# PaddlePaddle/MetaGym

Hardware: NVIDIA H100
Metric: env-steps/sec (quadrotor 6-DoF, 65k envs) (higher is better)
Workload: dtype f32

## Files before the change

### metagym_b200/csrc/quad.cu

```cuda
#include <math.h>
#include <stdlib.h>
#include <string.h>
#include <new>
#include <vector>

#include "mgb_common.cuh"
#include "quad_lanes.cuh"

namespace {

constexpr int kThreads = 64;
constexpr int kMaxObs = 19;

struct QuadConst {
    float h;
    float k1phi;
    float k1;
    float inv_phi;
    float hjm;
    float hk;
    float mm;
    float ct0, ct1, ct2;
    float vmin, vmax;
    float A[4], B[4];
    float px[4], py[4], pz[4];
    float Df[3], Dm[3];
    float cg[3];
    float hI[9];
    float gm;
    float c_hm;
    float c_h2m;
    float fail_r2, fail_v2, fail_w2;
    float dt, healthy, z_off;
    float init_v[3], init_w[3], noise_v, noise_w;
    int nt, task, substeps, obs_dim;
    int rk4_steps;
    float rk4_h;
    float inv_jm, inv_m;
    float Iinv[9];
    int simple;
};

struct QuadArgs {
    float4 *planes;
    int64_t n_pad;
    int64_t n;
    int64_t env_base;
    const float *act;
    float *obs;
    float *rew;
    uint8_t *done;
    int32_t *fail;
    float *final_obs;
    const float *targets;
    const int32_t *sat;
    int map_rows, map_cols, x_off, y_off;
    const int32_t *env2task;
    uint64_t seed;
    int auto_reset;
    int per_cta;
    int T;
    uint64_t act_seed;
    uint32_t t_base;
    float *act_out;
    MgbMirrors mir;
};

template <class T> struct VState {
    T p[3], v[3], om[3], w[4], R[9];
    int ct[Lanes<T>::N], ep[Lanes<T>::N];
};
using QState = VState<float>;

constexpr int kTileEnvs = 128;
constexpr int kPlanes = 6;

__device__ __forceinline__ float4 *tile_base(const QuadArgs &a, int64_t e)
{
    return a.planes + (e / kTileEnvs) * (kPlanes * kTileEnvs) + (e % kTileEnvs);
}

__device__ __forceinline__ void unpack_state(const float4 q[kPlanes], QState &s)
{
    s.p[0] = q[0].x; s.p[1] = q[0].y; s.p[2] = q[0].z; s.v[0] = q[0].w;
    s.v[1] = q[1].x; s.v[2] = q[1].y; s.om[0] = q[1].z; s.om[1] = q[1].w;
    s.om[2] = q[2].x; s.w[0] = q[2].y; s.w[1] = q[2].z; s.w[2] = q[2].w;
    s.w[3] = q[3].x; s.R[0] = q[3].y; s.R[1] = q[3].z; s.R[2] = q[3].w;
    s.R[3] = q[4].x; s.R[4] = q[4].y; s.R[5] = q[4].z; s.R[6] = q[4].w;
    s.R[7] = q[5].x; s.R[8] = q[5].y; s.ct[0] = __float_as_int(q[5].z); s.ep[0] = __float_as_int(q[5].w);
}
__device__ __forceinline__ void pack_state(const QState &s, float4 q[kPlanes])
{
    q[0] = make_float4(s.p[0], s.p[1], s.p[2], s.v[0]);
    q[1] = make_float4(s.v[1], s.v[2], s.om[0], s.om[1]);
    q[2] = make_float4(s.om[2], s.w[0], s.w[1], s.w[2]);
    q[3] = make_float4(s.w[3], s.R[0], s.R[1], s.R[2]);
    q[4] = make_float4(s.R[3], s.R[4], s.R[5], s.R[6]);
    q[5] = make_float4(s.R[7], s.R[8], __int_as_float(s.ct[0]), __int_as_float(s.ep[0]));
}

__device__ __forceinline__ void load_state(const QuadArgs &a, int64_t e, QState &s)
{
    const float4 *b = tile_base(a, e);
    float4 q[kPlanes];
#pragma unroll
    for (int k = 0; k < kPlanes; ++k) q[k] = b[k * kTileEnvs];
    unpack_state(q, s);
}

__device__ __forceinline__ void store_state(const QuadArgs &a, int64_t e, const QState &s)
{
    float4 *b = tile_base(a, e);
    float4 q[kPlanes];
    pack_state(s, q);
#pragma unroll
    for (int k = 0; k < kPlanes; ++k) b[k * kTileEnvs] = q[k];
}

template <class T> __device__ __forceinline__ void get_lane_state(const VState<T> &s, int h, QState &o);
template <class T> __device__ __forceinline__ void set_lane_state(VState<T> &s, int h, const QState &o);

__device__ __forceinline__ void load_state2(const QuadArgs &a, int64_t e, VState<f2> &s)
{
    QState s0, s1;
    load_state(a, e, s0);
    load_state(a, e + 1, s1);
    set_lane_state(s, 0, s0);
    set_lane_state(s, 1, s1);
}
__device__ __forceinline__ void store_state2(const QuadArgs &a, int64_t e, const VState<f2> &s)
{
    QState s0, s1;
    get_lane_state(s, 0, s0);
    get_lane_state(s, 1, s1);
    store_state(a, e, s0);
    store_state(a, e + 1, s1);
}
// ... 321 lines not shown
        for (int r = 0; r < 3; ++r) { acc.p[r] = fmaf(2.f, k.p[r], acc.p[r]); acc.v[r] = fmaf(2.f, k.v[r], acc.v[r]); acc.om[r] = fmaf(2.f, k.om[r], acc.om[r]); }
#pragma unroll
        for (int r = 0; r < 4; ++r) acc.w[r] = fmaf(2.f, k.w[r], acc.w[r]);
#pragma unroll
        for (int r = 0; r < 9; ++r) acc.R[r] = fmaf(2.f, k.R[r], acc.R[r]);
        quad_axpy(s, k, h, t);
        quad_rhs<SIMPLE>(c, t, kV, k);
#pragma unroll
        for (int r = 0; r < 3; ++r) { acc.p[r] += k.p[r]; acc.v[r] += k.v[r]; acc.om[r] += k.om[r]; }
#pragma unroll
        for (int r = 0; r < 4; ++r) acc.w[r] += k.w[r];
#pragma unroll
        for (int r = 0; r < 9; ++r) acc.R[r] += k.R[r];
        const int ct = s.ct[0], ep = s.ep[0];
        quad_axpy(s, acc, h * (1.0f / 6.0f), t);
        s = t; s.ct[0] = ct; s.ep[0] = ep;
        const float psq = sq3(s.p);
        const float vsq = sq3(s.v);
        const float osq = sq3(s.om);
        fail = fail_code(c, psq, vsq, osq);
        if (fail) break;
    }
    adjugate(s.R, adj, id);
    float pw = 0.f;
#pragma unroll
    for (int i = 0; i < 4; ++i) pw += fabsf(fmaf(-c.k1phi, s.w[i], kV[i]) * c.inv_phi * V[i]);
    power = pw;
    return fail;
}

template <class T>
__device__ __forceinline__ void observe(const QuadConst &c, const VState<T> &s, const T adj[9], T id, T *o, T bv[3],
                                        T Ri[9])
{
#pragma unroll
    for (int k = 0; k < 9; ++k) Ri[k] = vmul(adj[k], id);
#pragma unroll
    for (int r = 0; r < 3; ++r) {
        bv[r] = dot3(Ri[3 * r], s.v[0], Ri[3 * r + 1], s.v[1], Ri[3 * r + 2], s.v[2]);
        o[r] = bv[r];
        o[3 + r] = dot3(Ri[3 * r], s.p[0], Ri[3 * r + 1], s.p[1], Ri[3 * r + 2], s.p[2]);
        o[6 + r] = vmul(Ri[3 * r + 2], -9.8f);
        o[9 + r] = s.om[r];
    }
    o[12] = fast_atan2(vneg(s.R[6]), vsqrt(vfma(s.R[8], s.R[8], vmul(s.R[7], s.R[7]))));
    o[13] = fast_atan2(s.R[7], s.R[8]);
    o[14] = fast_atan2(s.R[3], s.R[0]);
    o[15] = vadd(s.p[2], c.z_off);
}

template <class T> __device__ __forceinline__ void reset_env(const QuadConst &c, VState<T> &s, int h, const double u[12])
{
#pragma unroll
    for (int k = 0; k < 3; ++k) {
        set_lane(s.p[k], h, 0.f);
        const double sv = u[k] > 0.5 ? 1.0 : -1.0, sw = u[6 + k] > 0.5 ? 1.0 : -1.0;
        set_lane(s.v[k], h, (float)((double)c.init_v[k] + ((double)c.noise_v * u[3 + k]) * sv));
        set_lane(s.om[k], h, (float)((double)c.init_w[k] + ((double)c.noise_w * u[9 + k]) * sw));
    }
#pragma unroll
    for (int k = 0; k < 4; ++k) set_lane(s.w[k], h, 0.f);
#pragma unroll
    for (int k = 0; k < 9; ++k) set_lane(s.R[k], h, (k % 4 == 0) ? 1.f : 0.f);
}

__device__ __forceinline__ void philox_reset_draws(uint64_t seed, int64_t genv, int ep, double u[12])
{
    const uint2 key = make_uint2((uint32_t)seed, (uint32_t)(seed >> 32));
#pragma unroll
    for (int j = 0; j < 3; ++j) {
        const uint4 r = mgb_philox4x32_10(
            make_uint4((uint32_t)genv, (uint32_t)((uint64_t)genv >> 32), (uint32_t)ep, MGB_STREAM_RESET + j), key);
        u[4 * j + 0] = (double)mgb_u01(r.x);
        u[4 * j + 1] = (double)mgb_u01(r.y);
        u[4 * j + 2] = (double)mgb_u01(r.z);
        u[4 * j + 3] = (double)mgb_u01(r.w);
    }
}

template <class T> struct TargetRows {
    T cur[3];
    T nxt[3];
};
template <class T>
__device__ __forceinline__ void prefetch_targets(const QuadConst &c, const float *trow, int ct, int h, TargetRows<T> &tr)
{
    const int t = ct < c.nt - 1 ? ct : c.nt - 1;
    const float *g = trow + 3 * (ct - 1), *q = trow + 3 * t;
    set_lane(tr.cur[0], h, __ldg(g)); set_lane(tr.cur[1], h, __ldg(g + 1)); set_lane(tr.cur[2], h, __ldg(g + 2));
    set_lane(tr.nxt[0], h, __ldg(q)); set_lane(tr.nxt[1], h, __ldg(q + 1)); set_lane(tr.nxt[2], h, __ldg(q + 2));
}

__device__ __forceinline__ int slice_bound(double v, int len)
{
    long long x = v < -2.0e9 ? -2000000000LL : (v > 2.0e9 ? 2000000000LL : (long long)v);
    if (x < 0) { x += len; if (x < 0) x = 0; }
    if (x > len) x = len;
    return (int)x;
}

__device__ __forceinline__ bool map_collision(const QuadArgs &a, float x_old, float y_old, float z_old, float x_new,
                                              float y_new, float z_new)
{
    const double xo = (double)x_old + a.x_off, xn = (double)x_new + a.x_off;
    const double yo = (double)y_old + a.y_off, yn = (double)y_new + a.y_off;
    const double x_min = floor(fmin(xo, xn)), x_max = ceil(fmax(xo, xn));
    const double y_min = floor(fmin(yo, yn)), y_max = ceil(fmax(yo, yn));
    const int z_lo = (int)floorf(fminf(z_old, z_new)), z_hi = (int)ceilf(fmaxf(z_old, z_new));
    const int ys = slice_bound(y_min, a.map_rows), ye = slice_bound(y_max + 1.0, a.map_rows);
    const int xs = slice_bound(x_min, a.map_cols), xe = slice_bound(x_max + 1.0, a.map_cols);
    int any = 0;
    if (ys < ye && xs < xe) {
        const int W = a.map_cols + 1;
        any = (a.sat[ye * W + xe] - a.sat[ys * W + xe] - a.sat[ye * W + xs] + a.sat[ys * W + xs]) > 0 ? 1 : 0;
    }
    return z_lo < any || z_hi < any;
}

template <class T>
__device__ __forceinline__ void observe_reset(const QuadConst &c, const QuadArgs &a, int64_t e, const VState<T> &s, int h,
                                              T *o)
{
    set_lane(o[0], h, lane(s.v[0], h)); set_lane(o[1], h, lane(s.v[1], h)); set_lane(o[2], h, lane(s.v[2], h));
    set_lane(o[3], h, 0.f); set_lane(o[4], h, 0.f); set_lane(o[5], h, 0.f);
    set_lane(o[6], h, 0.f * -9.8f); set_lane(o[7], h, 0.f * -9.8f); set_lane(o[8], h, -9.8f);
    set_lane(o[9], h, lane(s.om[0], h)); set_lane(o[10], h, lane(s.om[1], h)); set_lane(o[11], h, lane(s.om[2], h));
    set_lane(o[12], h, -0.f); set_lane(o[13], h, 0.f); set_lane(o[14], h, 0.f);
    set_lane(o[15], h, 0.f + c.z_off);
    if (c.task == MGB_TASK_VELOCITY_CONTROL) {
        const float *trow = a.targets + ((int64_t)a.env2task[e] * c.nt) * 3;
        const int t = s.ct[h] < c.nt - 1 ? s.ct[h] : c.nt - 1;
        set_lane(o[16], h, __ldg(trow + 3 * t)); set_lane(o[17], h, __ldg(trow + 3 * t + 1));
        set_lane(o[18], h, __ldg(trow + 3 * t + 2));
    }
}

template <class T>
__device__ __forceinline__ void finish_step(const QuadConst &c, const QuadArgs &a, int64_t e, VState<T> &s,
                                            const T adj[9], T id, T z_old, T x_old, T y_old, T power,
                                            const int fail[Lanes<T>::N], const TargetRows<T> &tr, T *o, T &reward,
                                            int done_flag[Lanes<T>::N], bool write_final[Lanes<T>::N])
{
    constexpr int N = Lanes<T>::N;
    T bv[3], Ri[9];
    observe(c, s, adj, id, o, bv, Ri);
    if (c.task == MGB_TASK_VELOCITY_CONTROL) {
        o[16] = tr.nxt[0]; o[17] = tr.nxt[1]; o[18] = tr.nxt[2];
    }
    reward = vneg(vmin(vmul(c.dt, power), bc<T>(c.healthy)));
    int done[N];
#pragma unroll
    for (int h = 0; h < N; ++h) done[h] = 0;
    if (c.task == MGB_TASK_VELOCITY_CONTROL) {
        const T g0 = tr.cur[0], g1 = tr.cur[1], g2 = tr.cur[2];
        T diff = bc<T>(0.f);
#pragma unroll
        for (int r = 0; r < 3; ++r) diff = vadd(diff, vabs(vsub(dot3(Ri[3 * r], g0, Ri[3 * r + 1], g1, Ri[3 * r + 2], g2), bv[r])));
        reward = vadd(reward, vmul(-0.001f, diff));
    } else {
        const T z_new = vadd(s.p[2], c.z_off);
        T bonus, vn, on;
        if (c.task == MGB_TASK_HOVERING_CONTROL) {
            vn = vsqrt(sq3(s.v));
            on = vsqrt(sq3(s.om));
        }
#pragma unroll
        for (int h = 0; h < N; ++h) {
            bool coll;
            if (a.sat) coll = map_collision(a, lane(x_old, h), lane(y_old, h), lane(z_old, h), lane(s.p[0], h),
                                            lane(s.p[1], h), lane(z_new, h));
            else coll = fminf(lane(z_old, h), lane(z_new, h)) < 0.f;
            float tr = coll ? 0.f : c.healthy;
            if (c.task == MGB_TASK_HOVERING_CONTROL) {
                tr -= lane(vn, h) + lane(on, h);
                const float zm = fabsf(0.f - lane(s.p[2], h));
                tr += zm < 0.5f ? 10.f : fmaxf(-20.f, 0.5f - zm);
            }
            set_lane(bonus, h, tr);
            if (coll) { done[h] = 1; s.ct[h] = 0; }
        }
        reward = vadd(reward, bonus);
    }
#pragma unroll
    for (int h = 0; h < N; ++h) {
        if (s.ct[h] == c.nt) { done[h] = 1; s.ct[h] = 0; }
        if (fail[h]) { done[h] = 1; s.ct[h] = 0; }
        done_flag[h] = done[h];
        write_final[h] = false;
        if (done[h] && a.auto_reset) {
            write_final[h] = true;
            s.ep[h] += 1;
            double u[12];
            philox_reset_draws(a.seed, a.env_base + e + h, s.ep[h], u);
            reset_env(c, s, h, u);
        }
    }
}

__device__ __forceinline__ void publish_tile(float *gobs, const float *tile, int64_t e0, int rows, int D)
{
    const uint32_t bytes = (uint32_t)rows * (uint32_t)D * 4u;
    float *dst = gobs + e0 * D;
    if ((bytes & 15u) == 0 && ((reinterpret_cast<uintptr_t>(dst) & 15u) == 0)) {
        mgb_fence_proxy_async();
        __syncthreads();
        if (threadIdx.x == 0) {
            mgb_bulk_store(dst, tile, bytes);
            mgb_bulk_commit();
        }
    } else {
        __syncthreads();
        for (int i = threadIdx.x; i < rows * D; i += blockDim.x) dst[i] = tile[i];
    }
}

__device__ __forceinline__ void publish_tile_mirrored(const MgbMirrors &m, float *gobs, const float *tile, int64_t e0,
                                                      int rows, int D)
{
    const uint32_t bytes = (uint32_t)rows * (uint32_t)D * 4u;
    float *dst = gobs + e0 * D;
    if ((bytes & 15u) == 0 && ((reinterpret_cast<uintptr_t>(dst) & 15u) == 0)) {
        mgb_fence_proxy_async();
        __syncthreads();
        if (threadIdx.x == 0) {
            mgb_bulk_store(dst, tile, bytes);
            mgb_mirror_bulk_store(m, dst, tile, bytes);
            mgb_bulk_commit();
        }
    } else {
        __syncthreads();
        for (int i = threadIdx.x; i < rows * D; i += blockDim.x) {
            dst[i] = tile[i];
            mgb_mirror_store(m, dst + i, tile[i]);
        }
    }
}

template <bool SIMPLE, bool EARLY, class T>
__device__ __forceinline__ void step_body(const QuadConst &c, const QuadArgs &a, int64_t e, int nact, VState<T> &s,
                                          const T V[4], float *trow, float *frow, int &final_mask)
{
    constexpr int N = Lanes<T>::N;
    const int D = c.obs_dim;
    T adj[9], id, power;
    adjugate(s.R, adj, id);
    TargetRows<T> tr;
    int ct_now[N];
#pragma unroll
    for (int h = 0; h < N; ++h) {
        s.ct[h] += 1;
        ct_now[h] = s.ct[h];
    }
    const bool vel = c.task == MGB_TASK_VELOCITY_CONTROL;
    if (EARLY && vel) {
#pragma unroll
        for (int h = 0; h < N; ++h) {
            const int64_t eh = h < nact ? e + h : e;
            prefetch_targets(c, a.targets + ((int64_t)__ldg(a.env2task + eh) * c.nt) * 3, ct_now[h], h, tr);
        }
    }
    const T z_old = vadd(s.p[2], c.z_off);
    const T x_old = s.p[0], y_old = s.p[1];
    int fail[N];
    if (N == 1 && c.rk4_steps > 0) {
        QState s1;
        get_lane_state(s, 0, s1);
        float adj1[9], id1, pw1;
        fail[0] = integrate_rk4<SIMPLE>(c, s1, make_float4(lane(V[0], 0), lane(V[1], 0), lane(V[2], 0), lane(V[3], 0)),
                                        adj1, id1, pw1);
        set_lane_state(s, 0, s1);
#pragma unroll
        for (int k = 0; k < 9; ++k) set_lane(adj[k], 0, adj1[k]);
        set_lane(id, 0, id1);
        set_lane(power, 0, pw1);
    } else {
        const bool failed = integrate<SIMPLE, T>(c, s, V, adj, id, power, fail);
        if (N > 1 && failed) {
#pragma unroll 1
            for (int h = 0; h < N; ++h) {
                QState s1;
                load_state(a, e + h, s1);
                float adj1[9], id1, pw1;
                adjugate(s1.R, adj1, id1);
                const float V1[4] = {lane(V[0], h), lane(V[1], h), lane(V[2], h), lane(V[3], h)};
                int f1[1];
                integrate<SIMPLE, float>(c, s1, V1, adj1, id1, pw1, f1);
                s1.ct[0] = s.ct[h];
                s1.ep[0] = s.ep[h];
                set_lane_state(s, h, s1);
#pragma unroll
                for (int k = 0; k < 9; ++k) set_lane(adj[k], h, adj1[k]);
                set_lane(id, h, id1);
                set_lane(power, h, pw1);
                fail[h] = f1[0];
            }
        }
    }
    if (!EARLY && vel) {
#pragma unroll
        for (int h = 0; h < N; ++h) {
            const int64_t eh = h < nact ? e + h : e;
            prefetch_targets(c, a.targets + ((int64_t)__ldg(a.env2task + eh) * c.nt) * 3, ct_now[h], h, tr);
        }
    }
    const bool state_first = N == 1 && !EARLY && vel;
    if (state_first) {
        QState s1;
        get_lane_state(s, 0, s1);
        if (s1.ct[0] == c.nt || fail[0]) s1.ct[0] = 0;
        store_state(a, e, s1);
    }
    T o[kMaxObs], reward;
    int done[N];
    bool wf[N];
    finish_step(c, a, e, s, adj, id, z_old, x_old, y_old, power, fail, tr, o, reward, done, wf);
    bool stored = false;
    if constexpr (N == 2) {
        if (nact == 2) {
            store_state2(a, e, s);
            *reinterpret_cast<float2 *>(a.rew + e) = reward.v;
            *reinterpret_cast<uchar2 *>(a.done + e) = make_uchar2((uint8_t)done[0], (uint8_t)done[1]);
            if (a.fail) *reinterpret_cast<int2 *>(a.fail + e) = make_int2(fail[0], fail[1]);
            stored = true;
        }
    }
    if (!stored) {
#pragma unroll
        for (int h = 0; h < N; ++h) {
            if (h < nact) {
                QState s1;
                get_lane_state(s, h, s1);
                if (!state_first || wf[h]) store_state(a, e + h, s1);
                a.rew[e + h] = lane(reward, h);
                a.done[e + h] = (uint8_t)done[h];
                if (a.fail) a.fail[e + h] = fail[h];
            }
        }
    }
#pragma unroll
    for (int h = 0; h < N; ++h) {
        if (h < nact) {
            float *tr_h = trow + h * D;
            if (wf[h]) {
                if (a.final_obs) {
                    float *fr_h = frow + h * D;
#pragma unroll
                    for (int k = 0; k < 16; ++k) fr_h[k] = lane(o[k], h);
                    if (D == 19) { fr_h[16] = lane(o[16], h); fr_h[17] = lane(o[17], h); fr_h[18] = lane(o[18], h); }
                    final_mask |= 1 << h;
                }
                observe_reset(c, a, e + h, s, h, o);
            }
#pragma unroll
            for (int k = 0; k < 16; ++k) tr_h[k] = lane(o[k], h);
            if (D == 19) { tr_h[16] = lane(o[16], h); tr_h[17] = lane(o[17], h); tr_h[18] = lane(o[18], h); }
        }
    }
}

__device__ __forceinline__ void publish_final(const QuadArgs &a, const float *ftile, int64_t e, int local_row, int lanes,
                                              int final_mask, int D)
{
    if (!a.final_obs) return;
    if (__syncthreads_or(final_mask)) {
        for (int h = 0; h < lanes; ++h) {
            if (final_mask & (1 << h)) {
                float *dst = a.final_obs + (e + h) * D;
                const float *frow = ftile + (local_row + h) * D;
                for (int k = 0; k < D; ++k) dst[k] = frow[k];
            }
        }
    }
}

template <bool SIMPLE>
__global__ void __launch_bounds__(kThreads) quad_step_kernel(const __grid_constant__ QuadConst c,
                                                             const __grid_constant__ QuadArgs a)
{
    __shared__ __align__(128) float tile[kThreads * kMaxObs];
    __shared__ __align__(128) float ftile[kThreads * kMaxObs];
    const int64_t e0 = (int64_t)blockIdx.x * kThreads;
    const int64_t e = e0 + threadIdx.x;
    const int rows = (int)((a.n - e0) < kThreads ? (a.n - e0) : kThreads);
    const int D = c.obs_dim;
    const bool active = e < a.n;
    int final_mask = 0;

    asm volatile("griddepcontrol.launch_dependents;");
    asm volatile("griddepcontrol.wait;" ::: "memory");

    if (active) {
        QState s;
        load_state(a, e, s);
        const float4 act = __ldg(reinterpret_cast<const float4 *>(a.act) + e);
        const float V[4] = {act.x, act.y, act.z, act.w};
        step_body<SIMPLE, false, float>(c, a, e, 1, s, V, tile + threadIdx.x * D, ftile + threadIdx.x * D, final_mask);
    }
    publish_tile(a.obs, tile, e0, rows, D);
    publish_final(a, ftile, e, threadIdx.x, 1, final_mask, D);
    if (threadIdx.x == 0) mgb_bulk_wait_read<0>();
}

template <bool SIMPLE>
__global__ void __launch_bounds__(512, 1) quad_step_wide_kernel(const __grid_constant__ QuadConst c,
                                                                const __grid_constant__ QuadArgs a)
{
    extern __shared__ __align__(128) float wide_smem[];
    const int per = a.per_cta;
    float *tile = wide_smem, *ftile = wide_smem + (size_t)per * kMaxObs;
    const int64_t e0 = (int64_t)blockIdx.x * per;
    const int64_t e = e0 + threadIdx.x;
    int rows = (int)((a.n - e0) < per ? (a.n - e0) : per);
    if (rows < 0) rows = 0;
    const int D = c.obs_dim;
    const bool active = (int)threadIdx.x < rows;
    int final_mask = 0;
    asm volatile("griddepcontrol.launch_dependents;");
    asm volatile("griddepcontrol.wait;" ::: "memory");
    if (active) {
        QState s;
        load_state(a, e, s);
        const float4 act = __ldg(reinterpret_cast<const float4 *>(a.act) + e);
        const float V[4] = {act.x, act.y, act.z, act.w};
        step_body<SIMPLE, true, float>(c, a, e, 1, s, V, tile + threadIdx.x * D, ftile + threadIdx.x * D, final_mask);
    }
    if (rows > 0) publish_tile(a.obs, tile, e0, rows, D);
    else __syncthreads();
    publish_final(a, ftile, e, threadIdx.x, 1, final_mask, D);
    if (threadIdx.x == 0) mgb_bulk_wait_read<0>();
}

template <bool SIMPLE>
__global__ void __launch_bounds__(256, 1) quad_step2_kernel(const __grid_constant__ QuadConst c,
                                                            const __grid_constant__ QuadArgs a)
{
    extern __shared__ __align__(128) float pair_smem[];
    const int per = a.per_cta;
    float *tile = pair_smem, *ftile = pair_smem + (size_t)per * kMaxObs;
    const int64_t e0 = (int64_t)blockIdx.x * per;
    int rows = (int)((a.n - e0) < per ? (a.n - e0) : per);
    if (rows < 0) rows = 0;
    const int le = 2 * (int)threadIdx.x;
    const int64_t e = e0 + le;
    const int D = c.obs_dim;
    const int nact = rows - le >= 2 ? 2 : (rows - le > 0 ? 1 : 0);
    int final_mask = 0;
    asm volatile("griddepcontrol.launch_dependents;");
    asm volatile("griddepcontrol.wait;" ::: "memory");
    if (nact > 0) {
        VState<f2> s;
        load_state2(a, e, s);
        const float4 a0 = __ldg(reinterpret_cast<const float4 *>(a.act) + e);
        const float4 a1 = nact == 2 ? __ldg(reinterpret_cast<const float4 *>(a.act) + e + 1) : make_float4(0.f, 0.f, 0.f, 0.f);
        const f2 V[4] = {pack2(a0.x, a1.x), pack2(a0.y, a1.y), pack2(a0.z, a1.z), pack2(a0.w, a1.w)};
        step_body<SIMPLE, true, f2>(c, a, e, nact, s, V, tile + le * D, ftile + le * D, final_mask);
    }
    if (rows > 0) publish_tile(a.obs, tile, e0, rows, D);
    else __syncthreads();
    publish_final(a, ftile, e, le, 2, final_mask, D);
    if (threadIdx.x == 0) mgb_bulk_wait_read<0>();
}

constexpr int kStreamThreads = 128;

template <bool SIMPLE>
__global__ void __launch_bounds__(kStreamThreads, 4) quad_stream_kernel(const __grid_constant__ QuadConst c,
                                                                        const __grid_constant__ QuadArgs a)
{
    __shared__ __align__(128) float4 stage[2][7][kStreamThreads];
    __shared__ __align__(128) float tile[kStreamThreads * kMaxObs];
    __shared__ __align__(128) float ftile[kStreamThreads * kMaxObs];
    __shared__ __align__(8) uint64_t full[2];
    const int D = c.obs_dim;
    const int64_t n_tiles = (a.n + kStreamThreads - 1) / kStreamThreads;
    const int tid = threadIdx.x;

    asm volatile("griddepcontrol.launch_dependents;");
    asm volatile("griddepcontrol.wait;" ::: "memory");
    if (tid == 0) {
        mgb_mbar_init(&full[0], 1);
        mgb_mbar_init(&full[1], 1);
        mgb_fence_mbar_init();
    }
    __syncthreads();

    auto fetch = [&](int64_t t, int st) {
        const int64_t e0 = t * kStreamThreads;
        const uint32_t rows = (uint32_t)((a.n - e0) < kStreamThreads ? (a.n - e0) : kStreamThreads);
        static_assert(kStreamThreads == kTileEnvs, "one CTA iteration = one state tile");
        mgb_mbar_expect_tx(&full[st], 6u * kTileEnvs * 16u + rows * 16u);
        mgb_bulk_load(stage[st][0], a.planes + t * (6 * kTileEnvs), 6u * kTileEnvs * 16u, &full[st]);
        mgb_bulk_load(stage[st][6], reinterpret_cast<const float4 *>(a.act) + e0, rows * 16u, &full[st]);
    };

    int64_t t = blockIdx.x;
    if (tid == 0 && t < n_tiles) fetch(t, 0);
    uint32_t phase[2] = {0u, 0u};
    int st = 0;
    for (; t < n_tiles; t += gridDim.x, st ^= 1) {
        const int64_t t_next = t + gridDim.x;
        if (tid == 0 && t_next < n_tiles) fetch(t_next, st ^ 1);
        mgb_mbar_wait(&full[st], phase[st]);
        phase[st] ^= 1u;
        const int64_t e0 = t * kStreamThreads, e = e0 + tid;
        const int rows = (int)((a.n - e0) < kStreamThreads ? (a.n - e0) : kStreamThreads);
        int final_mask = 0;
        if (tid == 0) mgb_bulk_wait_read<0>();
        __syncthreads();
        if (tid < rows) {
            QState s;
            float4 q[kPlanes];
#pragma unroll
            for (int k = 0; k < kPlanes; ++k) q[k] = stage[st][k][tid];
            unpack_state(q, s);
            const float4 act = stage[st][6][tid];
            const float V[4] = {act.x, act.y, act.z, act.w};
            step_body<SIMPLE, true, float>(c, a, e, 1, s, V, tile + tid * D, ftile + tid * D, final_mask);
        }
        publish_tile(a.obs, tile, e0, rows, D);
        publish_final(a, ftile, e, tid, 1, final_mask, D);
        __syncthreads();
    }
    if (tid == 0) mgb_bulk_wait_read<0>();
}

template <bool SIMPLE, int XM>
__global__ void __launch_bounds__(kThreads, 8) quad_rollout_kernel(const __grid_constant__ QuadConst c,
                                                                const __grid_constant__ QuadArgs a)
{
    __shared__ __align__(128) float tiles[2][kThreads * kMaxObs];
    const int64_t e0 = (int64_t)blockIdx.x * kThreads;
    const int64_t e = e0 + threadIdx.x;
    const int rows = (int)((a.n - e0) < kThreads ? (a.n - e0) : kThreads);
    const int D = c.obs_dim;
    const bool active = e < a.n;
    QState s;
    float adj[9], id = 1.f;
    if (active) {
        load_state(a, e, s);
        adjugate(s.R, adj, id);
    }
    const uint2 akey = make_uint2((uint32_t)a.act_seed, (uint32_t)(a.act_seed >> 32));
    const int64_t genv = a.env_base + e;
    const float *trow = nullptr;
    if (active && c.task == MGB_TASK_VELOCITY_CONTROL) trow = a.targets + ((int64_t)__ldg(a.env2task + e) * c.nt) * 3;
    float4 act_next = make_float4(0.f, 0.f, 0.f, 0.f);
    if (active && a.act) act_next = __ldg(reinterpret_cast<const float4 *>(a.act) + e);
    for (int t = 0; t < a.T; ++t) {
        float *tile = tiles[t & 1];
        if (threadIdx.x == 0) mgb_bulk_wait_read<1>();
        __syncthreads();
        uint32_t done_byte = 0;
        if (active) {
            float4 act;
            if (a.act) {
                act = act_next;
                if (t + 1 < a.T) act_next = __ldg(reinterpret_cast<const float4 *>(a.act) + (int64_t)(t + 1) * a.n + e);
            } else {
                const uint4 r = mgb_philox4x32_10(make_uint4((uint32_t)genv, (uint32_t)((uint64_t)genv >> 32),
                                                             a.t_base + (uint32_t)t, MGB_STREAM_ACTION),
                                                  akey);
                const float span = c.vmax - c.vmin;
                act = make_float4(fmaf(span, mgb_u01(r.x), c.vmin), fmaf(span, mgb_u01(r.y), c.vmin),
                                  fmaf(span, mgb_u01(r.z), c.vmin), fmaf(span, mgb_u01(r.w), c.vmin));
                if (a.act_out) {
                    float4 *ap = reinterpret_cast<float4 *>(a.act_out) + (int64_t)t * a.n + e;
                    if (XM == 2) mgb_mc_st(mgb_shift(ap, a.mir.delta[0]), act);
                    else *ap = act;
                    if (XM == 1) mgb_mirror_store(a.mir, ap, act);
                }
            }
            s.ct[0] += 1;
            TargetRows<float> tr;
            if (c.task == MGB_TASK_VELOCITY_CONTROL) prefetch_targets(c, trow, s.ct[0], 0, tr);
            const float z_old = s.p[2] + c.z_off;
            const float x_old = s.p[0], y_old = s.p[1];
            float power;
            int fail[1];
            fail[0] = integrate1<SIMPLE>(c, s, act, adj, id, power);
            float o[kMaxObs], reward;
            int done[1];
            bool wf[1];
            finish_step<float>(c, a, e, s, adj, id, z_old, x_old, y_old, power, fail, tr, o, reward, done, wf);
            if (wf[0]) {
                observe_reset(c, a, e, s, 0, o);
                adjugate(s.R, adj, id);
            }
            if (a.rew) {
                if (XM == 2) mgb_mc_st(mgb_shift(a.rew + (int64_t)t * a.n + e, a.mir.delta[0]), reward);
                else a.rew[(int64_t)t * a.n + e] = reward;
                if (XM == 1) mgb_mirror_store(a.mir, a.rew + (int64_t)t * a.n + e, reward);
            }
            done_byte = (uint32_t)done[0];
            if (a.done && XM != 2) {
                a.done[(int64_t)t * a.n + e] = (uint8_t)done[0];
                if (XM == 1) mgb_mirror_store(a.mir, a.done + (int64_t)t * a.n + e, (uint8_t)done[0]);
            }
            if (a.obs) {
                float *orow = tile + threadIdx.x * D;
#pragma unroll
                for (int k = 0; k < 16; ++k) orow[k] = o[k];
                if (D == 19) { orow[16] = o[16]; orow[17] = o[17]; orow[18] = o[18]; }
            }
        }
        if (XM == 2) {
            if (a.done) mgb_mc_st_bytes(mgb_shift(a.done + (int64_t)t * a.n + e, a.mir.delta[0]), done_byte, active);
            if (a.obs) {
                __syncthreads();
                mgb_mc_copy_tile(mgb_shift(a.obs + ((int64_t)t * a.n + e0) * D, a.mir.delta[0]), tile,
                                 (uint32_t)rows * (uint32_t)D * 4u);
            }
        } else if (a.obs) {
            if (XM == 1) publish_tile_mirrored(a.mir, a.obs + (int64_t)t * a.n * D, tile, e0, rows, D);
            else publish_tile(a.obs + (int64_t)t * a.n * D, tile, e0, rows, D);
        }
    }
    if (active) store_state(a, e, s);
    if (threadIdx.x == 0) mgb_bulk_wait_read<0>();
}

__global__ void __launch_bounds__(kThreads) quad_reset_kernel(const __grid_constant__ QuadConst c,
                                                              const __grid_constant__ QuadArgs a,
                                                              const uint8_t *__restrict__ mask,
                                                              const double *__restrict__ noise)
{
    const int64_t e = (int64_t)blockIdx.x * kThreads + threadIdx.x;
    if (e >= a.n) return;
    QState s;
    load_state(a, e, s);
    if (!mask || mask[e]) {
        double u[12];
        if (noise) {
#pragma unroll
            for (int k = 0; k < 12; ++k) u[k] = noise[e * 12 + k];
        } else {
            s.ep[0] += 1;
            philox_reset_draws(a.seed, a.env_base + e, s.ep[0], u);
        }
        reset_env(c, s, 0, u);
        store_state(a, e, s);
    }
    if (a.obs) {
        float adj[9], id, o[kMaxObs], bv[3], Ri[9];
        adjugate(s.R, adj, id);
        observe(c, s, adj, id, o, bv, Ri);
        if (c.task == MGB_TASK_VELOCITY_CONTROL) {
            const float *trow = a.targets + ((int64_t)a.env2task[e] * c.nt) * 3;
            const int t = s.ct[0] < c.nt - 1 ? s.ct[0] : c.nt - 1;
            o[16] = trow[3 * t]; o[17] = trow[3 * t + 1]; o[18] = trow[3 * t + 2];
        }
        float *dst = a.obs + e * c.obs_dim;
#pragma unroll
        for (int k = 0; k < 16; ++k) dst[k] = o[k];
        if (c.obs_dim == 19) { dst[16] = o[16]; dst[17] = o[17]; dst[18] = o[18]; }
    }
}

__global__ void quad_state_kernel(QuadArgs a, float *state, int32_t *ct, int load)
{
    const int64_t e = (int64_t)blockIdx.x * blockDim.x + threadIdx.x;
    if (e >= a.n) return;
    QState s;
    load_state(a, e, s);
    float *row = state + e * 22;
    if (load) {
        for (int k = 0; k < 3; ++k) { s.p[k] = row[k]; s.v[k] = row[3 + k]; s.om[k] = row[6 + k]; }
        for (int k = 0; k < 4; ++k) s.w[k] = row[9 + k];
        for (int k = 0; k < 9; ++k) s.R[k] = row[13 + k];
        if (ct) s.ct[0] = ct[e];
        store_state(a, e, s);
    } else {
        for (int k = 0; k < 3; ++k) { row[k] = s.p[k]; row[3 + k] = s.v[k]; row[6 + k] = s.om[k]; }
        for (int k = 0; k < 4; ++k) row[9 + k] = s.w[k];
        for (int k = 0; k < 9; ++k) row[13 + k] = s.R[k];
        if (ct) ct[e] = s.ct[0];
    }
}

__global__ void quad_init_kernel(QuadArgs a)
{
    const int64_t e = (int64_t)blockIdx.x * blockDim.x + threadIdx.x;
    if (e >= a.n_pad) return;
    QState s;
    for (int k = 0; k < 3; ++k) s.p[k] = s.v[k] = s.om[k] = 0.f;
    for (int k = 0; k < 4; ++k) s.w[k] = 0.f;
    for (int k = 0; k < 9; ++k) s.R[k] = (k % 4 == 0) ? 1.f : 0.f;
    s.ct[0] = 0;
    s.ep[0] = 0;
    store_state(a, e, s);
}

template <bool SIMPLE>
__global__ void quad_targets_kernel(const __grid_constant__ QuadConst c, const float *__restrict__ act, int n_tasks,
                                    float *__restrict__ tbl)
{
    const int k = blockIdx.x * blockDim.x + threadIdx.x;
    if (k >= n_tasks) return;
    QState s;
    for (int q = 0; q < 3; ++q) s.p[q] = s.v[q] = s.om[q] = 0.f;
    for (int q = 0; q < 4; ++q) s.w[q] = 0.f;
    for (int q = 0; q < 9; ++q) s.R[q] = (q % 4 == 0) ? 1.f : 0.f;
    s.ct[0] = 0; s.ep[0] = 0;
    float adj[9], id, power;
    adjugate(s.R, adj, id);
    for (int t = 0; t < c.nt; ++t) {
        const float4 a4 = reinterpret_cast<const float4 *>(act)[(int64_t)k * c.nt + t];
        const int fail = integrate1<SIMPLE>(c, s, a4, adj, id, power);
        float *dst = tbl + ((int64_t)k * c.nt + t) * 3;
        dst[0] = s.v[0]; dst[1] = s.v[1]; dst[2] = s.v[2];
        if (fail) {
            for (int r = t + 1; r < c.nt; ++r) {
                float *d2 = tbl + ((int64_t)k * c.nt + r) * 3;
                d2[0] = d2[1] = d2[2] = __int_as_float(0x7fc00000);
            }
            return;
        }
    }
}

}

struct mgb_quad {
    int device = 0;
    int64_t n = 0, n_pad = 0, env_base = 0;
    mgb_quad_cfg cfg;
    QuadConst c;
    float4 *planes = nullptr;
    int32_t *sat = nullptr;
    int map_rows = 0, map_cols = 0, x_off = 0, y_off = 0;
    float *targets = nullptr;
    int32_t *env2task = nullptr;
    int n_tasks = 0;
    int auto_reset = 0;
    int num_sms = 132;
    int wide_kernel = -1;
    int packed = 0;
    int stream_kernel = 1;
    int pdl = 1;
    int zerocopy = 1;
    uint64_t seed = 0;
    uint32_t t_base = 0;
    int64_t launches = 0;
    MgbMirrors mir = {};
    MgbMirrorWindow mir_win;
    float *h_act = nullptr, *h_obs = nullptr, *h_rew = nullptr, *h_final = nullptr;
    uint8_t *h_done = nullptr;
    int32_t *h_fail = nullptr;
    float *d_act = nullptr, *d_obs = nullptr, *d_rew = nullptr, *d_final = nullptr;
    uint8_t *d_done = nullptr;
    int32_t *d_fail = nullptr;
};

static QuadArgs base_args(const mgb_quad *h)
{
    QuadArgs a;
    memset(&a, 0, sizeof(a));
    a.planes = h->planes;
    a.n_pad = h->n_pad;
    a.n = h->n;
    a.env_base = h->env_base;
    a.targets = h->targets;
    a.sat = h->sat; a.map_rows = h->map_rows; a.map_cols = h->map_cols; a.x_off = h->x_off; a.y_off = h->y_off;
    a.env2task = h->env2task;
    a.seed = h->seed;
    a.auto_reset = h->auto_reset;
    return a;
}

static int derive_constants(const mgb_quad_cfg *g, QuadConst *c)
{
    memset(c, 0, sizeof(*c));
    c->h = (float)g->precision;
    c->k1 = (float)(g->phi / g->ra);
    c->k1phi = (float)(g->phi / g->ra * g->phi);
    c->inv_phi = (float)(1.0 / g->phi);
    c->hjm = (float)(g->precision / g->jm);
    c->hk = (float)(g->precision / g->jm * (g->phi / g->ra * g->phi));
    c->mm = (float)g->mm;
    c->ct0 = (float)g->ct[0]; c->ct1 = (float)g->ct[1]; c->ct2 = (float)g->ct[2];
    c->vmin = (float)g->min_voltage; c->vmax = (float)g->max_voltage;
    bool simple = (g->ct[2] == 0.0);
    for (int i = 0; i < 4; ++i) {
        c->px[i] = g->propeller[3 * i]; c->py[i] = g->propeller[3 * i + 1]; c->pz[i] = g->propeller[3 * i + 2];
        c->A[i] = (float)((double)c->py[i] * (double)g->propeller_norm[i]);
        c->B[i] = (float)((double)c->px[i] * (double)g->propeller_norm[i]);
        if (c->pz[i] != 0.f) simple = false;
    }
    for (int k = 0; k < 3; ++k) {
        c->Df[k] = g->drag_f[k]; c->Dm[k] = g->drag_m[k]; c->cg[k] = g->gravity_center[k];
        if (c->cg[k] != 0.f) simple = false;
        c->init_v[k] = g->init_velocity[k]; c->init_w[k] = g->init_angular_velocity[k];
    }
    for (int k = 0; k < 9; ++k) {
        c->hI[k] = (float)(g->precision * (double)g->inv_inertia[k]);
        if (k % 4 != 0 && g->inv_inertia[k] != 0.f) simple = false;
    }
    c->gm = (float)((double)(float)-9.8 * g->quality);
    c->c_hm = (float)(g->precision / g->quality);
    c->c_h2m = (float)(0.5 * g->precision * g->precision / g->quality);
    c->fail_r2 = (float)(g->fail_range * g->fail_range);
    c->fail_v2 = (float)(g->fail_velocity * g->fail_velocity);
    c->fail_w2 = (float)(g->fail_w * g->fail_w);
    c->dt = (float)g->dt; c->healthy = (float)g->healthy_reward; c->z_off = (float)g->z_offset;
    c->noise_v = (float)g->init_velocity_noise; c->noise_w = (float)g->init_angular_velocity_noise;
    c->nt = g->nt; c->task = g->task;
    c->substeps = (int)(g->dt / g->precision);
    c->rk4_steps = g->integrator == MGB_INTEGRATOR_RK4 ? (g->rk4_steps > 0 ? g->rk4_steps : 1) : 0;
    c->rk4_h = c->rk4_steps ? (float)(g->dt / c->rk4_steps) : 0.f;
    c->inv_jm = (float)(1.0 / g->jm);
    c->inv_m = (float)(1.0 / g->quality);
    for (int k = 0; k < 9; ++k) c->Iinv[k] = g->inv_inertia[k];
    c->obs_dim = g->task == MGB_TASK_VELOCITY_CONTROL ? 19 : 16;
    c->simple = simple ? 1 : 0;
    return 0;
}

extern "C" int mgb_quad_create(mgb_quad **out, int64_t n_envs, const mgb_quad_cfg *cfg, int device,
                               int64_t env_index_base)
{
    MGB_REQUIRE(out && cfg, "null argument");
    MGB_REQUIRE(n_envs > 0, "n_envs must be positive");
    MGB_REQUIRE(cfg->task >= 0 && cfg->task <= 2, "invalid task");
    MGB_REQUIRE(cfg->nt > 0, "nt must be positive");
    MGB_REQUIRE(!(cfg->precision < 1e-8 || cfg->precision > cfg->dt), "Inproper parameter of precision");
    int ndev = 0;
    MGB_CUDA(cudaGetDeviceCount(&ndev));
    MGB_REQUIRE(device >= 0 && device < ndev, "device index out of range");
    MgbDeviceGuard guard(device);
    mgb_quad *h = new (std::nothrow) mgb_quad();
    MGB_REQUIRE(h, "out of host memory");
    h->device = device;
    h->n = n_envs;
    h->n_pad = (n_envs + 127) / 128 * 128;
    h->env_base = env_index_base;
    h->cfg = *cfg;
    derive_constants(cfg, &h->c);
    if (const char *ev = getenv("MGB_PDL")) h->pdl = atoi(ev) != 0;
    {
        cudaDeviceProp prop;
        if (cudaGetDeviceProperties(&prop, device) == cudaSuccess) h->num_sms = prop.multiProcessorCount;
    }
    if (const char *ev = getenv("MGB_HOST_ZEROCOPY")) h->zerocopy = atoi(ev);
    if (const char *ev = getenv("MGB_STREAM_KERNEL")) h->stream_kernel = atoi(ev) != 0;
    if (const char *ev = getenv("MGB_PACKED")) h->packed = atoi(ev) != 0;
// ... 15 lines not shown
        mgb_set_error("cudaMalloc(state planes, %lld envs) -> %s", (long long)n_envs, cudaGetErrorString(e));
        delete h;
        return MGB_ERR_CUDA;
    }
    QuadArgs a = base_args(h);
    quad_init_kernel<<<(unsigned)((h->n_pad + 255) / 256), 256>>>(a);
    e = cudaDeviceSynchronize();
    if (e != cudaSuccess) {
        mgb_set_error("state init -> %s", cudaGetErrorString(e));
        cudaFree(h->planes);
        delete h;
        return MGB_ERR_CUDA;
    }
    h->launches += 1;
    *out = h;
    return MGB_OK;
}

extern "C" void mgb_quad_destroy(mgb_quad *h)
{
    if (!h) return;
    MgbDeviceGuard guard(h->device);
    cudaDeviceSynchronize();
    cudaFree(h->planes);
    cudaFree(h->sat);
    cudaFree(h->targets);
    cudaFree(h->env2task);
    cudaFree(h->d_act); cudaFree(h->d_obs); cudaFree(h->d_rew); cudaFree(h->d_done);
    cudaFree(h->d_fail); cudaFree(h->d_final);
    cudaFreeHost(h->h_act); cudaFreeHost(h->h_obs); cudaFreeHost(h->h_rew); cudaFreeHost(h->h_done);
    cudaFreeHost(h->h_fail); cudaFreeHost(h->h_final);
    delete h;
}

extern "C" int mgb_quad_obs_dim(const mgb_quad *h) { return h ? h->c.obs_dim : MGB_ERR_ARG; }
extern "C" int64_t mgb_quad_num_envs(const mgb_quad *h) { return h ? h->n : MGB_ERR_ARG; }
extern "C" int64_t mgb_quad_launch_count(const mgb_quad *h) { return h ? h->launches : MGB_ERR_ARG; }

extern "C" int mgb_quad_set_options(mgb_quad *h, int auto_reset, uint64_t seed)
{
    MGB_REQUIRE(h, "null handle");
    h->auto_reset = auto_reset ? 1 : 0;
    h->seed = seed;
    return MGB_OK;
}

extern "C" int mgb_quad_set_map(mgb_quad *h, const int32_t *map_host, int32_t rows, int32_t cols)
{
    MGB_REQUIRE(h, "null handle");
    MgbDeviceGuard guard(h->device);
    MGB_CUDA(cudaDeviceSynchronize());
    cudaFree(h->sat);
    h->sat = nullptr;
    h->map_rows = h->map_cols = h->x_off = h->y_off = 0;
    if (!map_host) return MGB_OK;
    MGB_REQUIRE(h->c.task != MGB_TASK_VELOCITY_CONTROL, "velocity_control has no map (env.py:101-104)");
    MGB_REQUIRE(rows > 0 && cols > 0 && rows <= 8192 && cols <= 8192, "map size out of range");
    int starts = 0, sr = 0, sc = 0;
    for (int r = 0; r < rows; ++r)
        for (int q = 0; q < cols; ++q)
            if (map_host[(size_t)r * cols + q] == -1) { ++starts; sr = r; sc = q; }
    MGB_REQUIRE(starts == 1, "the map must mark exactly one start cell with -1 (env.py:108-109)");
    std::vector<int32_t> sat((size_t)(rows + 1) * (cols + 1), 0);
    for (int r = 0; r < rows; ++r)
        for (int q = 0; q < cols; ++q) {
            const int v = (r == sr && q == sc) ? 0 : map_host[(size_t)r * cols + q];
            sat[(size_t)(r + 1) * (cols + 1) + q + 1] = (v != 0 ? 1 : 0) + sat[(size_t)r * (cols + 1) + q + 1] +
                                                        sat[(size_t)(r + 1) * (cols + 1) + q] - sat[(size_t)r * (cols + 1) + q];
        }
    MGB_CUDA(cudaMalloc(&h->sat, sat.size() * sizeof(int32_t)));
    MGB_CUDA(cudaMemcpy(h->sat, sat.data(), sat.size() * sizeof(int32_t), cudaMemcpyHostToDevice));
    h->map_rows = rows; h->map_cols = cols; h->x_off = sc; h->y_off = sr;
    return MGB_OK;
}

extern "C" int mgb_quad_set_targets(mgb_quad *h, const float *tbl_dev, int32_t n_tasks, const int32_t *env2task_dev)
{
    MGB_REQUIRE(h && tbl_dev && env2task_dev, "null argument");
    MGB_REQUIRE(n_tasks > 0, "n_tasks must be positive");
    MgbDeviceGuard guard(h->device);
    MGB_CUDA(cudaDeviceSynchronize());
    cudaFree(h->targets); h->targets = nullptr;
    cudaFree(h->env2task); h->env2task = nullptr;
    const size_t tb = sizeof(float) * 3 * (size_t)h->c.nt * (size_t)n_tasks;
    MGB_CUDA(cudaMalloc(&h->targets, tb));
    MGB_CUDA(cudaMalloc(&h->env2task, sizeof(int32_t) * h->n));
    MGB_CUDA(cudaMemcpy(h->targets, tbl_dev, tb, cudaMemcpyDeviceToDevice));
    MGB_CUDA(cudaMemcpy(h->env2task, env2task_dev, sizeof(int32_t) * h->n, cudaMemcpyDeviceToDevice));
    MGB_CUDA(cudaDeviceSynchronize());
    h->n_tasks = n_tasks;
    return MGB_OK;
}

static int check_ready(const mgb_quad *h)
{
    if (h->c.task == MGB_TASK_VELOCITY_CONTROL && !h->targets) {
        mgb_set_error("velocity_control: call mgb_quad_set_targets before reset/step");
        return MGB_ERR_STATE;
    }
    return MGB_OK;
}

extern "C" int mgb_quad_make_targets(mgb_quad *h, const float *act_dev, int32_t n_tasks, float *tbl_dev, void *stream)
{
    MgbRange nvtx_range("mgb_quad_make_targets");
    MGB_REQUIRE(h && act_dev && tbl_dev, "null argument");
    MGB_REQUIRE(n_tasks > 0, "n_tasks must be positive");
    MgbDeviceGuard guard(h->device);
    cudaStream_t st = (cudaStream_t)stream;
    const int threads = 32, blocks = (n_tasks + threads - 1) / threads;
    if (h->c.simple) quad_targets_kernel<true><<<blocks, threads, 0, st>>>(h->c, act_dev, n_tasks, tbl_dev);
    else quad_targets_kernel<false><<<blocks, threads, 0, st>>>(h->c, act_dev, n_tasks, tbl_dev);
    MGB_CUDA(cudaGetLastError());
    h->launches += 1;
    return MGB_OK;
}

extern "C" int mgb_quad_reset(mgb_quad *h, const uint8_t *mask_dev, const double *noise_dev, float *obs_dev,
                              void *stream)
{
    MgbRange nvtx_range("mgb_quad_reset");
    MGB_REQUIRE(h, "null handle");
    int rc = check_ready(h);
    if (rc) return rc;
    MgbDeviceGuard guard(h->device);
    QuadArgs a = base_args(h);
    a.obs = obs_dev;
    quad_reset_kernel<<<(unsigned)((h->n + kThreads - 1) / kThreads), kThreads, 0, (cudaStream_t)stream>>>(
        h->c, a, mask_dev, noise_dev);
    MGB_CUDA(cudaGetLastError());
    h->launches += 1;
    return MGB_OK;
}

enum StepKernel { STEP_TILE = 0, STEP_WIDE = 1, STEP_STREAM = 2, STEP_PACKED = 3 };

static StepKernel choose_step_kernel(const mgb_quad *h, const QuadArgs &a)
{
    const unsigned blocks = (unsigned)((a.n + kThreads - 1) / kThreads);
    const bool act16 = (reinterpret_cast<uintptr_t>(a.act) & 15u) == 0;
    if (h->stream_kernel && (int64_t)blocks > (int64_t)h->num_sms * 32 && act16) return STEP_STREAM;
    if (h->packed && h->c.rk4_steps == 0 && a.n >= 2) {
        const bool aligned = act16 && (reinterpret_cast<uintptr_t>(a.rew) & 7u) == 0 &&
                             (reinterpret_cast<uintptr_t>(a.done) & 1u) == 0 && (reinterpret_cast<uintptr_t>(a.fail) & 7u) == 0;
        if (aligned) return STEP_PACKED;
    }
    const bool single_wave = a.n <= (int64_t)h->num_sms * 512 && a.n >= (int64_t)h->num_sms * 64;
    const int64_t wide_max = (int64_t)h->num_sms * (h->wide_kernel > 0 ? 512 : 384);
    if (h->wide_kernel != 0 && single_wave && a.n <= wide_max) return STEP_WIDE;
    return STEP_TILE;
}

static int launch_step(mgb_quad *h, const QuadArgs &a, cudaStream_t st)
{
    const unsigned blocks = (unsigned)((a.n + kThreads - 1) / kThreads);
    cudaLaunchConfig_t cfg;
    memset(&cfg, 0, sizeof(cfg));
    cfg.gridDim = dim3(blocks);
    cfg.blockDim = dim3(kThreads);
    cfg.stream = st;
    cudaLaunchAttribute attr[1];
    attr[0].id = cudaLaunchAttributeProgrammaticStreamSerialization;
    attr[0].val.programmaticStreamSerializationAllowed = h->pdl ? 1 : 0;
    cfg.attrs = attr;
    cfg.numAttrs = 1;
    const StepKernel which = choose_step_kernel(h, a);
    if (which == STEP_STREAM) {
        cfg.gridDim = dim3((unsigned)(h->num_sms * 4));
        cfg.blockDim = dim3(kStreamThreads);
        if (h->c.simple) MGB_CUDA(cudaLaunchKernelEx(&cfg, quad_stream_kernel<true>, h->c, a));
// ... 228 lines not shown
```

Baseline: 8.507 billion.

## Store velocity targets as time-major float4 rows and hoist env2task lookup

Target tables are converted at set time into a time-major, task-minor float4 layout, so each target row is read with a single vector load and envs sharing a step index hit nearby addresses. The env-to-task index is now loaded once per thread before griddepcontrol.wait instead of inside every prefetch. The step kernels also change which template path they use: one kernel drops early prefetch, a STATE_FIRST flag is added, and the fused loop moves the prefetch after integration. The float4 layout uses a third more target memory and needs an extra layout kernel when targets are set.

```diff
diff --git a/metagym_b200/csrc/quad.cu b/metagym_b200/csrc/quad.cu
--- a/metagym_b200/csrc/quad.cu
+++ b/metagym_b200/csrc/quad.cu
@@ -52,7 +52,8 @@
     uint8_t *done;
     int32_t *fail;
     float *final_obs;
-    const float *targets;
+    const float4 *targets;
+    int n_tasks;
     const int32_t *sat;
     int map_rows, map_cols, x_off, y_off;
     const int32_t *env2task;
@@ -540,13 +541,22 @@
     T cur[3];
     T nxt[3];
 };
+__device__ __forceinline__ float4 target_row(const QuadArgs &a, int task, int t)
+{
+    return __ldg(a.targets + (int64_t)t * a.n_tasks + task);
+}
 template <class T>
-__device__ __forceinline__ void prefetch_targets(const QuadConst &c, const float *trow, int ct, int h, TargetRows<T> &tr)
+__device__ __forceinline__ void prefetch_targets(const QuadConst &c, const QuadArgs &a, int task, int ct, int h,
+                                                 TargetRows<T> &tr)
 {
     const int t = ct < c.nt - 1 ? ct : c.nt - 1;
-    const float *g = trow + 3 * (ct - 1), *q = trow + 3 * t;
-    set_lane(tr.cur[0], h, __ldg(g)); set_lane(tr.cur[1], h, __ldg(g + 1)); set_lane(tr.cur[2], h, __ldg(g + 2));
-    set_lane(tr.nxt[0], h, __ldg(q)); set_lane(tr.nxt[1], h, __ldg(q + 1)); set_lane(tr.nxt[2], h, __ldg(q + 2));
+    const float4 g = target_row(a, task, ct - 1), q = target_row(a, task, t);
+    set_lane(tr.cur[0], h, g.x); set_lane(tr.cur[1], h, g.y); set_lane(tr.cur[2], h, g.z);
+    set_lane(tr.nxt[0], h, q.x); set_lane(tr.nxt[1], h, q.y); set_lane(tr.nxt[2], h, q.z);
+}
+__device__ __forceinline__ int env_task(const QuadConst &c, const QuadArgs &a, int64_t e)
+{
+    return c.task == MGB_TASK_VELOCITY_CONTROL ? __ldg(a.env2task + e) : 0;
 }
 
 __device__ __forceinline__ int slice_bound(double v, int len)
@@ -576,7 +586,7 @@
 }
 
 template <class T>
-__device__ __forceinline__ void observe_reset(const QuadConst &c, const QuadArgs &a, int64_t e, const VState<T> &s, int h,
+__device__ __forceinline__ void observe_reset(const QuadConst &c, const QuadArgs &a, int task, const VState<T> &s, int h,
                                               T *o)
 {
     set_lane(o[0], h, lane(s.v[0], h)); set_lane(o[1], h, lane(s.v[1], h)); set_lane(o[2], h, lane(s.v[2], h));
@@ -586,10 +596,8 @@
     set_lane(o[12], h, -0.f); set_lane(o[13], h, 0.f); set_lane(o[14], h, 0.f);
     set_lane(o[15], h, 0.f + c.z_off);
     if (c.task == MGB_TASK_VELOCITY_CONTROL) {
-        const float *trow = a.targets + ((int64_t)a.env2task[e] * c.nt) * 3;
-        const int t = s.ct[h] < c.nt - 1 ? s.ct[h] : c.nt - 1;
-        set_lane(o[16], h, __ldg(trow + 3 * t)); set_lane(o[17], h, __ldg(trow + 3 * t + 1));
-        set_lane(o[18], h, __ldg(trow + 3 * t + 2));
+        const float4 q = target_row(a, task, s.ct[h] < c.nt - 1 ? s.ct[h] : c.nt - 1);
+        set_lane(o[16], h, q.x); set_lane(o[17], h, q.y); set_lane(o[18], h, q.z);
     }
 }
 
@@ -694,9 +702,10 @@
     }
 }
 
-template <bool SIMPLE, bool EARLY, class T>
+template <bool SIMPLE, bool EARLY, bool STATE_FIRST, class T>
 __device__ __forceinline__ void step_body(const QuadConst &c, const QuadArgs &a, int64_t e, int nact, VState<T> &s,
-                                          const T V[4], float *trow, float *frow, int &final_mask)
+                                          const T V[4], const int task[Lanes<T>::N], float *trow, float *frow,
+                                          int &final_mask)
 {
     constexpr int N = Lanes<T>::N;
     const int D = c.obs_dim;
@@ -712,10 +721,7 @@
     const bool vel = c.task == MGB_TASK_VELOCITY_CONTROL;
     if (EARLY && vel) {
 #pragma unroll
-        for (int h = 0; h < N; ++h) {
-            const int64_t eh = h < nact ? e + h : e;
-            prefetch_targets(c, a.targets + ((int64_t)__ldg(a.env2task + eh) * c.nt) * 3, ct_now[h], h, tr);
-        }
+        for (int h = 0; h < N; ++h) prefetch_targets(c, a, task[h], ct_now[h], h, tr);
     }
     const T z_old = vadd(s.p[2], c.z_off);
     const T x_old = s.p[0], y_old = s.p[1];
@@ -756,12 +762,9 @@
     }
     if (!EARLY && vel) {
 #pragma unroll
-        for (int h = 0; h < N; ++h) {
-            const int64_t eh = h < nact ? e + h : e;
-            prefetch_targets(c, a.targets + ((int64_t)__ldg(a.env2task + eh) * c.nt) * 3, ct_now[h], h, tr);
-        }
-    }
-    const bool state_first = N == 1 && !EARLY && vel;
+        for (int h = 0; h < N; ++h) prefetch_targets(c, a, task[h], ct_now[h], h, tr);
+    }
+    const bool state_first = N == 1 && STATE_FIRST && vel;
     if (state_first) {
         QState s1;
         get_lane_state(s, 0, s1);
@@ -807,7 +810,7 @@
                     if (D == 19) { fr_h[16] = lane(o[16], h); fr_h[17] = lane(o[17], h); fr_h[18] = lane(o[18], h); }
                     final_mask |= 1 << h;
                 }
-                observe_reset(c, a, e + h, s, h, o);
+                observe_reset(c, a, task[h], s, h, o);
             }
 #pragma unroll
             for (int k = 0; k < 16; ++k) tr_h[k] = lane(o[k], h);
@@ -845,6 +848,7 @@
     int final_mask = 0;
 
     asm volatile("griddepcontrol.launch_dependents;");
+    const int task[1] = {active ? env_task(c, a, e) : 0};
     asm volatile("griddepcontrol.wait;" ::: "memory");
 
     if (active) {
@@ -852,7 +856,8 @@
         load_state(a, e, s);
         const float4 act = __ldg(reinterpret_cast<const float4 *>(a.act) + e);
         const float V[4] = {act.x, act.y, act.z, act.w};
-        step_body<SIMPLE, false, float>(c, a, e, 1, s, V, tile + threadIdx.x * D, ftile + threadIdx.x * D, final_mask);
+        step_body<SIMPLE, false, true, float>(c, a, e, 1, s, V, task, tile + threadIdx.x * D, ftile + threadIdx.x * D,
+                                              final_mask);
     }
     publish_tile(a.obs, tile, e0, rows, D);
     publish_final(a, ftile, e, threadIdx.x, 1, final_mask, D);
@@ -874,13 +879,15 @@
     const bool active = (int)threadIdx.x < rows;
     int final_mask = 0;
     asm volatile("griddepcontrol.launch_dependents;");
+    const int task[1] = {active ? env_task(c, a, e) : 0};
     asm volatile("griddepcontrol.wait;" ::: "memory");
     if (active) {
         QState s;
         load_state(a, e, s);
         const float4 act = __ldg(reinterpret_cast<const float4 *>(a.act) + e);
         const float V[4] = {act.x, act.y, act.z, act.w};
-        step_body<SIMPLE, true, float>(c, a, e, 1, s, V, tile + threadIdx.x * D, ftile + threadIdx.x * D, final_mask);
+        step_body<SIMPLE, false, false, float>(c, a, e, 1, s, V, task, tile + threadIdx.x * D, ftile + threadIdx.x * D,
+                                               final_mask);
     }
     if (rows > 0) publish_tile(a.obs, tile, e0, rows, D);
     else __syncthreads();
@@ -911,7 +918,8 @@
         const float4 a0 = __ldg(reinterpret_cast<const float4 *>(a.act) + e);
         const float4 a1 = nact == 2 ? __ldg(reinterpret_cast<const float4 *>(a.act) + e + 1) : make_float4(0.f, 0.f, 0.f, 0.f);
         const f2 V[4] = {pack2(a0.x, a1.x), pack2(a0.y, a1.y), pack2(a0.z, a1.z), pack2(a0.w, a1.w)};
-        step_body<SIMPLE, true, f2>(c, a, e, nact, s, V, tile + le * D, ftile + le * D, final_mask);
+        const int task[2] = {env_task(c, a, e), env_task(c, a, nact == 2 ? e + 1 : e)};
+        step_body<SIMPLE, true, false, f2>(c, a, e, nact, s, V, task, tile + le * D, ftile + le * D, final_mask);
     }
     if (rows > 0) publish_tile(a.obs, tile, e0, rows, D);
     else __syncthreads();
@@ -973,7 +981,8 @@
             unpack_state(q, s);
             const float4 act = stage[st][6][tid];
             const float V[4] = {act.x, act.y, act.z, act.w};
-            step_body<SIMPLE, true, float>(c, a, e, 1, s, V, tile + tid * D, ftile + tid * D, final_mask);
+            const int task[1] = {env_task(c, a, e)};
+            step_body<SIMPLE, true, false, float>(c, a, e, 1, s, V, task, tile + tid * D, ftile + tid * D, final_mask);
         }
         publish_tile(a.obs, tile, e0, rows, D);
         publish_final(a, ftile, e, tid, 1, final_mask, D);
@@ -1000,8 +1009,7 @@
     }
     const uint2 akey = make_uint2((uint32_t)a.act_seed, (uint32_t)(a.act_seed >> 32));
     const int64_t genv = a.env_base + e;
-    const float *trow = nullptr;
-    if (active && c.task == MGB_TASK_VELOCITY_CONTROL) trow = a.targets + ((int64_t)__ldg(a.env2task + e) * c.nt) * 3;
+    const int task = active ? env_task(c, a, e) : 0;
     float4 act_next = make_float4(0.f, 0.f, 0.f, 0.f);
     if (active && a.act) act_next = __ldg(reinterpret_cast<const float4 *>(a.act) + e);
     for (int t = 0; t < a.T; ++t) {
@@ -1030,18 +1038,18 @@
             }
             s.ct[0] += 1;
             TargetRows<float> tr;
-            if (c.task == MGB_TASK_VELOCITY_CONTROL) prefetch_targets(c, trow, s.ct[0], 0, tr);
             const float z_old = s.p[2] + c.z_off;
             const float x_old = s.p[0], y_old = s.p[1];
             float power;
             int fail[1];
             fail[0] = integrate1<SIMPLE>(c, s, act, adj, id, power);
+            if (c.task == MGB_TASK_VELOCITY_CONTROL) prefetch_targets(c, a, task, s.ct[0], 0, tr);
             float o[kMaxObs], reward;
             int done[1];
             bool wf[1];
             finish_step<float>(c, a, e, s, adj, id, z_old, x_old, y_old, power, fail, tr, o, reward, done, wf);
             if (wf[0]) {
-                observe_reset(c, a, e, s, 0, o);
+                observe_reset(c, a, task, s, 0, o);
                 adjugate(s.R, adj, id);
             }
             if (a.rew) {
@@ -1103,9 +1111,8 @@
         adjugate(s.R, adj, id);
         observe(c, s, adj, id, o, bv, Ri);
         if (c.task == MGB_TASK_VELOCITY_CONTROL) {
-            const float *trow = a.targets + ((int64_t)a.env2task[e] * c.nt) * 3;
-            const int t = s.ct[0] < c.nt - 1 ? s.ct[0] : c.nt - 1;
-            o[16] = trow[3 * t]; o[17] = trow[3 * t + 1]; o[18] = trow[3 * t + 2];
+            const float4 q = target_row(a, env_task(c, a, e), s.ct[0] < c.nt - 1 ? s.ct[0] : c.nt - 1);
+            o[16] = q.x; o[17] = q.y; o[18] = q.z;
         }
         float *dst = a.obs + e * c.obs_dim;
 #pragma unroll
@@ -1176,6 +1183,15 @@
     }
 }
 
+__global__ void quad_targets_layout_kernel(const float *__restrict__ src, int nt, int n_tasks, float4 *__restrict__ dst)
+{
+    const int64_t i = (int64_t)blockIdx.x * blockDim.x + threadIdx.x;
+    if (i >= (int64_t)nt * n_tasks) return;
+    const int64_t t = i / n_tasks, k = i % n_tasks;
+    const float *s = src + (k * nt + t) * 3;
+    dst[i] = make_float4(s[0], s[1], s[2], 0.f);
+}
+
 }
 
 struct mgb_quad {
@@ -1186,7 +1202,7 @@
     float4 *planes = nullptr;
     int32_t *sat = nullptr;
     int map_rows = 0, map_cols = 0, x_off = 0, y_off = 0;
-    float *targets = nullptr;
+    float4 *targets = nullptr;
     int32_t *env2task = nullptr;
     int n_tasks = 0;
     int auto_reset = 0;
@@ -1218,6 +1234,7 @@
     a.n = h->n;
     a.env_base = h->env_base;
     a.targets = h->targets;
+    a.n_tasks = h->n_tasks;
     a.sat = h->sat; a.map_rows = h->map_rows; a.map_cols = h->map_cols; a.x_off = h->x_off; a.y_off = h->y_off;
     a.env2task = h->env2task;
     a.seed = h->seed;
@@ -1399,10 +1416,12 @@
     MGB_CUDA(cudaDeviceSynchronize());
     cudaFree(h->targets); h->targets = nullptr;
     cudaFree(h->env2task); h->env2task = nullptr;
-    const size_t tb = sizeof(float) * 3 * (size_t)h->c.nt * (size_t)n_tasks;
-    MGB_CUDA(cudaMalloc(&h->targets, tb));
+    h->n_tasks = 0;
+    const int64_t rows = (int64_t)h->c.nt * n_tasks;
+    MGB_CUDA(cudaMalloc(&h->targets, sizeof(float4) * (size_t)rows));
     MGB_CUDA(cudaMalloc(&h->env2task, sizeof(int32_t) * h->n));
-    MGB_CUDA(cudaMemcpy(h->targets, tbl_dev, tb, cudaMemcpyDeviceToDevice));
+    quad_targets_layout_kernel<<<(unsigned)((rows + 255) / 256), 256>>>(tbl_dev, h->c.nt, n_tasks, h->targets);
+    MGB_CUDA(cudaGetLastError());
     MGB_CUDA(cudaMemcpy(h->env2task, env2task_dev, sizeof(int32_t) * h->n, cudaMemcpyDeviceToDevice));
     MGB_CUDA(cudaDeviceSynchronize());
     h->n_tasks = n_tasks;
```

Measured after the change: 8.789 billion (median of 6 runs). 3.3% higher.
